# cvxgrp/qcqp

Measured on AMD Instinct MI355X. Metric: restarts x coord-sweeps / sec (improve COORD_DESCENT phase-2 sweeps, 2n^2 flops each; whole step timed), higher is better.
Workload: dtype f64

## Files before the change

qcqp_amd/csrc/capi.hip:

```cpp
#include <dlfcn.h>
#include <unistd.h>
#include <hip/hip_runtime.h>
#include <rccl/rccl.h>

#include <algorithm>
#include <cmath>
#include <cstdarg>
#include <cstdio>
#include <cstring>
#include <string>
#include <chrono>
#include <vector>

#include "../../include/qcqp_mi.h"
#include "kernels.hip"
#include "admm.h"
#include "admm_fused.h"
#include "cd_queue.h"
#include "cd_life.h"
#include "gemm_pk.h"
#include "cd_general.h"
#include "cd_dense.h"
#include "sdr_solve.h"

// ... 108 lines not shown
    char *h_pin = nullptr;
    size_t h_pin_cap = 0;
    int64_t out_cap = 0;
    int eval_zs = 1;
    double *d_wS = nullptr, *d_wY = nullptr, *d_ww = nullptr, *d_wz = nullptr;
    int64_t wY_cap = 0;
    double *d_planes = nullptr;
    int64_t planes_cap = 0;
    double *d_gP = nullptr;
    const double *dn_Gpack = nullptr, *dn_q = nullptr, *dn_qT = nullptr, *dn_r = nullptr;
    const int *dn_relop = nullptr;
    double *dn_G = nullptr, *dn_Dg = nullptr, *dn_Ft = nullptr;
    int dense_chain_mode = 0;
    long long *dn_prof = nullptr;
    int64_t dn_G_cap = 0, dn_state_cap = 0;
    void *dn_state = nullptr;
    hipStream_t stream2 = nullptr;
    hipEvent_t dn_ev[3] = {nullptr, nullptr, nullptr};
    hipEvent_t dn_evn[2] = {nullptr, nullptr};
    int *dn_hn = nullptr;
    bool dn_force = false;
    double stream_limit = 16e9;
    double *dn_gp_pre = nullptr, *dn_tmp = nullptr;
    ncclComm_t comm = nullptr;
    int rank = 0, world = 1;
    double *d_comm = nullptr, *d_comm_big = nullptr;
    int64_t comm_big_cap = 0;
    long long *d_prof = nullptr;
    int cd_stage = 0;
    int64_t Xi_cap = 0;
    bool sdr_factor_resident = false;
    double ad_Minv_rho = 0.0;
    bool ad_Minv_device = false;
    const char *last_cd2_kernel = "";
    bool profile = false;
    int dbg = 0;
    char *af_work = nullptr;
    size_t af_work_cap = 0;
    bool ad_fused = true;
    int ad_fused_nt = 512;
    const char *last_admm_kernel = "";
    int last_admm_C = 0;
    long long af_prof[16] = {0};
    int cd_queue = 2;
    int *d_qnext = nullptr;
    bool q_prepared = false;
    CdLife *d_life = nullptr;
    int Kreal = 0;
    double fbound = 0.0;
    double *l2_scratch = nullptr; size_t l2_scratch_cap = 0;
    double *l2_D = nullptr, *l2_S = nullptr;
    int *l2_abort = nullptr;
    int *l2_cuslot = nullptr;
    double *lr_L = nullptr, *lr_G = nullptr, *lr_U = nullptr; int lr_RB = 0;
    int life_version = 0;
    long long *d_life_prof = nullptr;
    int64_t *d_bestK_idx = nullptr; double *d_bestK_key = nullptr, *d_bestK_x = nullptr; int64_t bestK_cap = 0;
    bool cd_ref_order = false;
    bool force_generic = false;
    std::vector<int> last_st1, last_st2;
};

namespace {

void admm_free(qcqpmi_ctx *c, bool keep_zsolver);

int fail(qcqpmi_ctx *c, int code, const char *fmt, ...) {
    char buf[1024];
    va_list ap;
    va_start(ap, fmt);
    vsnprintf(buf, sizeof(buf), fmt, ap);
    va_end(ap);
    if (c) c->err = buf; else g_create_error = buf;
    return code;
}

#define HIPCHK(c, expr)                                                                       \
    do {                                                                                      \
        hipError_t e_ = (expr);                                                               \
        if (e_ != hipSuccess)                                                                 \
            return fail(c, QCQPMI_EHIP, "%s failed: %s (%s:%d)", #expr, hipGetErrorString(e_), \
                        __FILE__, __LINE__);                                                  \
    } while (0)

template <typename T>
int dev_alloc(qcqpmi_ctx *c, T **p, size_t count, bool zero = true) {
    void *v = nullptr;
    HIPCHK(c, hipMalloc(&v, std::max<size_t>(count, 1) * sizeof(T)));
    if (zero) HIPCHK(c, hipMemsetAsync(v, 0, std::max<size_t>(count, 1) * sizeof(T), c->stream));
    *p = (T *)v;
    return 0;
}

template <typename T>
int prob_upload(qcqpmi_ctx *c, const T **dst, const std::vector<T> &src) {
    T *p = nullptr;
    int rc = dev_alloc(c, &p, src.size(), false);
    if (rc) return rc;
    c->prob_allocs.push_back(p);
    if (!src.empty())
        HIPCHK(c, hipMemcpyAsync(p, src.data(), src.size() * sizeof(T), hipMemcpyHostToDevice, c->stream));
    *dst = p;
    return 0;
}

void free_population(qcqpmi_ctx *c) {
// ... 412 lines not shown
    if ((rc = cd_apply_status(c, st, st1, f0, maxviol, GEN_CAP))) return rc;
    return 0;
}


extern "C" {

int qcqpmi_abi_version(void) { return QCQPMI_ABI_VERSION; }

int qcqpmi_device_count(void) {
    int n = 0;
    if (hipGetDeviceCount(&n) != hipSuccess) return 0;
    return n;
}

const char *qcqpmi_last_error(const qcqpmi_ctx *ctx) {
    return ctx ? ctx->err.c_str() : g_create_error.c_str();
}

int qcqpmi_ctx_create(qcqpmi_ctx **out, int64_t n, int64_t m, int device) {
    if (!out || n <= 0 || m < 0) return fail(nullptr, QCQPMI_EINVAL, "ctx_create: bad arguments");
    int ndev = qcqpmi_device_count();
    if (ndev <= 0)
        return fail(nullptr, QCQPMI_EHIP, "no HIP device visible: the qcqp_amd engine requires an MI355X (there is no CPU fallback)");
    if (device < 0 || device >= ndev) return fail(nullptr, QCQPMI_EINVAL, "device %d out of range (%d visible)", device, ndev);
    qcqpmi_ctx *c = new qcqpmi_ctx();
    c->device = device; c->n = n; c->m = m; c->n16 = (n + 15) / 16 * 16;
    c->quads.resize((size_t)m + 1);
    if (const char *sl = getenv("QCQPMI_STREAM_LIMIT")) { const double v = atof(sl); if (v > 0.0) c->stream_limit = v; }
    hipError_t e = hipSetDevice(device);
    if (e == hipSuccess) e = hipStreamCreateWithFlags(&c->stream, hipStreamNonBlocking);
    for (int i = 0; i < 5 && e == hipSuccess; i++) {
        e = hipEventCreate(&c->timers[i].beg);
        if (e == hipSuccess) e = hipEventCreate(&c->timers[i].end);
    }
    if (e != hipSuccess) {
        int rc = fail(nullptr, QCQPMI_EHIP, "ctx_create: %s", hipGetErrorString(e));
        delete c;
        return rc;
    }
    *out = c;
    return 0;
}

void qcqpmi_ctx_destroy(qcqpmi_ctx *c) {
    if (!c) return;
    (void)hipSetDevice(c->device);
    if (c->stream) (void)spin_sync(c->stream);
    if (c->comm && rccl() && rccl()->CommDestroy) rccl()->CommDestroy(c->comm);
    free_population(c);
    admm_free(c, false);
    for (void *p : c->prob_allocs) (void)hipFree(p);
    void *ptrs[] = {c->d_Fpack, c->d_Frow, c->d_mu, c->d_best_idx, c->d_best_key, c->d_comm, c->d_comm_big,
                    c->dn_G, c->dn_Dg, c->dn_Ft, c->dn_prof, c->dn_state, c->d_planes, c->d_out, c->d_wS, c->d_wY, c->d_ww, c->d_wz, c->af_work, c->d_qnext, c->d_life, c->d_life_prof, c->d_bestK_idx, c->d_bestK_key, c->d_bestK_x, c->l2_scratch, c->l2_D, c->l2_S, c->l2_abort, c->l2_cuslot, c->lr_L, c->lr_G, c->lr_U};
    if (c->h_out) (void)hipHostFree(c->h_out);
    if (c->h_pin) (void)hipHostFree(c->h_pin);
    for (void *p : ptrs) if (p) (void)hipFree(p);
    for (auto &t : c->timers) { if (t.beg) (void)hipEventDestroy(t.beg); if (t.end) (void)hipEventDestroy(t.end); }
    for (auto &e : c->dn_ev) if (e) (void)hipEventDestroy(e);
    for (auto &e : c->dn_evn) if (e) (void)hipEventDestroy(e);
    if (c->dn_hn) (void)hipHostFree(c->dn_hn);
    if (c->stream2) (void)hipStreamDestroy(c->stream2);
    if (c->stream) (void)hipStreamDestroy(c->stream);
    delete c;
}

int qcqpmi_set_quad(qcqpmi_ctx *c, int64_t k, int format, const double *vals, const int64_t *idx,
                    const int64_t *ptr, int64_t nnz, const double *q, double r, int relop) {
    if (!c) return QCQPMI_EINVAL;
    if (c->finalized) return fail(c, QCQPMI_ESTATE, "set_quad after finalize");
    if (k < 0 || k > c->m || !q) return fail(c, QCQPMI_EINVAL, "set_quad: bad k or q");
    if ((k == 0) != (relop == 0) || relop < 0 || relop > 2)
        return fail(c, QCQPMI_EINVAL, "set_quad: relop %d invalid for function %lld", relop, (long long)k);
    HostQuad &h = c->quads[(size_t)k];
    h = HostQuad();
    const int64_t n = c->n;
    if (format == QCQPMI_FMT_DENSE) {
        if (!vals) return fail(c, QCQPMI_EINVAL, "set_quad: dense vals missing");
        for (int64_t i = 0; i < n; i++)
            for (int64_t j = 0; j < n; j++) {
                double v = vals[i * n + j];
                if (v != 0.0) { h.ci.push_back((int)i); h.cj.push_back((int)j); h.cv.push_back(v); }
            }
    } else if (format == QCQPMI_FMT_CSR) {
        if (!ptr || (nnz > 0 && (!idx || !vals))) return fail(c, QCQPMI_EINVAL, "set_quad: CSR arrays missing");
        for (int64_t i = 0; i < n; i++)
            for (int64_t e = ptr[i]; e < ptr[i + 1]; e++) {
                if (idx[e] < 0 || idx[e] >= n || e >= nnz) return fail(c, QCQPMI_EINVAL, "set_quad: CSR index out of range");
                if (vals[e] != 0.0) { h.ci.push_back((int)i); h.cj.push_back((int)idx[e]); h.cv.push_back(vals[e]); }
            }
    } else {
        return fail(c, QCQPMI_EINVAL, "set_quad: unknown format %d", format);
    }
    if (format == QCQPMI_FMT_DENSE) {
        for (int64_t i = 0; i < n; i++)
            for (int64_t j = i + 1; j < n; j++)
                if (vals[i * n + j] != vals[j * n + i])
                    return fail(c, QCQPMI_EINVAL, "set_quad: P of function %lld is not symmetric (entry %lld,%lld); pass (P + P^T)/2",
                                (long long)k, (long long)i, (long long)j);
    } else {
        std::vector<std::pair<int64_t, double>> ent(h.cv.size());
        for (size_t e = 0; e < h.cv.size(); e++) ent[e] = {(int64_t)h.ci[e] * n + h.cj[e], h.cv[e]};
        std::sort(ent.begin(), ent.end(), [](const std::pair<int64_t, double> &a, const std::pair<int64_t, double> &b) { return a.first < b.first; });
        size_t w = 0;
        for (size_t e = 0; e < ent.size(); e++) {
            if (w > 0 && ent[w - 1].first == ent[e].first) ent[w - 1].second += ent[e].second;
            else ent[w++] = ent[e];
// ... 686 lines not shown
        const size_t NB = (size_t)(c->n16 / 16);
        if ((rc = dev_alloc(c, &c->l2_D, NB * 256))) return rc;
        if ((rc = dev_alloc(c, &c->l2_S, NB * 48))) return rc;
        hipError_t e = (hipError_t)cd_life2_pack(c->dp, c->l2_D, c->l2_S, c->stream);
        if (e != hipSuccess) return fail(c, QCQPMI_EHIP, "cd_life2_pack: %s", hipGetErrorString(e));
    }
    return 0;
}

int qcqpmi_cd_stream_run(qcqpmi_ctx *c, int64_t K, int64_t R, int generate, int phase1, int64_t num_iters, double viol_tol, double tol,
                         uint64_t seed, uint64_t seed_stride, uint64_t first_index, uint64_t first_stride, double select_tol,
                         int64_t *sweeps1, int64_t *sweeps2, int64_t *visits2, int64_t *accepted2, uint8_t *ran_phase2, double *f0,
                         double *maxviol, int64_t *best_index, double *best_f0, double *best_maxviol, double *best_x) {
    int rc = check_ready(c, generate ? false : true);
    if (rc) return rc;
    if (K < 1 || R < 1 || num_iters < 0 || !(tol > 0.0) || K * R >= (1LL << 30)) return fail(c, QCQPMI_EINVAL, "cd_stream_run: bad K / R / num_iters / tol");
    if (!generate && c->R != K * R) return fail(c, QCQPMI_EINVAL, "cd_stream_run: the resident population has %lld points, K R = %lld", (long long)c->R, (long long)(K * R));
    HIPCHK(c, hipSetDevice(c->device));
    const bool stt = getenv("QCQPMI_STREAM_TIMING") != nullptr;
    double stm[6] = {0, 0, 0, 0, 0, 0};
    auto stnow = []() { return std::chrono::duration<double, std::milli>(std::chrono::steady_clock::now().time_since_epoch()).count(); };
    stm[0] = stnow();
    int nmw = 0, cs2 = 0, kind = 0;
    const int factor_rb = (c->lr_RB > 0 && c->life_version != 3 && cd_life2_factor_ok(c->dp, 16 * (int64_t)c->lr_RB)) ? c->lr_RB : 0;
    bool use2 = c->life_version != 1 && !c->force_generic && !(c->dbg & 64) && c->sep &&
                cd_life2_config(c->dp, c->Kreal, c->objclass, c->symcls, factor_rb, &nmw, &cs2, &kind);
    int cs = 0;
    const int queue_switch = c->cd_queue;
    c->cd_queue = 2;
    const bool eligible = cd_queue_eligible(c, false) && (int)(c->n16 / 16) - 4 <= RQ_NSIMD * RQ_MAXU && c->n16 >= 48;
    c->cd_queue = queue_switch;
    const bool lr = use2 && factor_rb > 0 && nmw == 3 && (kind == L2_KIND_BAND || kind == L2_KIND_GEN);
    if (lr) cs2 = 0;
    if (!use2) {
        if (!eligible || c->life_version != 1)
            return fail(c, QCQPMI_EUNSUPPORTED, "cd_stream_run: the lifecycle kernel needs separable constraints -- at most four classes of coordinates, at most two constraints "
                        "per coordinate --, a diagonal of P0 that is positive everywhere or zero everywhere, and 48 <= n <= 2304: use qcqpmi_cd_run per population");
        const int NBq = (int)(c->n16 / 16);
        cs = (c->dbg & 128) ? ((c->dbg >> 8) & 7) : 4;
        cs = cs > RQ_CSMAX ? RQ_CSMAX : cs;
        if (cs >= NBq) cs = 0;
        cs &= ~1;
        if (NBq - cs > RQ_NSIMD * RQ_MAXU || NBq < 3) return fail(c, QCQPMI_EUNSUPPORTED, "cd_stream_run: n = %lld outside the range of cd_phase2_qs_kernel (n <= 1024, at least 3 blocks of 16)", (long long)c->n);
    }
    if (generate && (rc = pop_reserve(c, K * R))) return rc;
    if (!c->d_qnext && (rc = dev_alloc(c, &c->d_qnext, 16))) return rc;
    if (!c->d_life) HIPCHK(c, hipMalloc((void **)&c->d_life, sizeof(CdLife)));
    HIPCHK(c, hipMemsetAsync(c->d_qnext, 0, 16 * sizeof(int), c->stream));
    CdLife L;
    L.on = 1; L.generate = generate ? 1 : 0; L.phase1 = phase1 ? 1 : 0; L.Rtotal = K * R; L.Rpop = R;
    L.seed = seed; L.seed_stride = seed_stride; L.first_index = first_index; L.first_stride = first_stride; L.viol_tol = viol_tol;
    L.sweeps1 = c->d_sweeps1; L.status1 = c->d_status1; L.ran2 = c->d_flag;
    L.prof = nullptr;
    if (c->profile) {
        if (!c->d_life_prof) HIPCHK(c, hipMalloc((void **)&c->d_life_prof, 24 * sizeof(long long)));
        HIPCHK(c, hipMemsetAsync(c->d_life_prof, 0, 24 * sizeof(long long), c->stream));
        L.prof = c->d_life_prof;
    }
    HIPCHK(c, hipMemcpyAsync(c->d_life, &L, sizeof(L), hipMemcpyHostToDevice, c->stream));
    HIPCHK(c, spin_sync(c->stream));
    int cus = 0;
    HIPCHK(c, hipDeviceGetAttribute(&cus, hipDeviceAttributeMultiprocessorCount, c->device));
    stm[1] = stnow();
    if (use2) {
        if ((rc = cd_life2_reserve(c, nmw, cus))) return rc;
        if (!lr && (c->dbg & 128)) { const int k2 = (c->dbg >> 8) & 7; if (nmw == 3 && (k2 == 0 || k2 == 2 || k2 == 4) && k2 < (int)(c->n16 / 16)) cs2 = k2; }
        const int tiles = cd_life2_tiles(c->dp, nmw, cs2, K * R, cus, 0, lr ? 1 : 0);
        int64_t wgs = (K * R + 16 * tiles - 1) / (16 * tiles);
        const int maxw = cd_life2_max_wgs(nmw, cus, tiles);
        if (wgs > maxw) wgs = maxw;
        if (c->dbg & 1024) { const int lim = (c->dbg >> 12) & 1023; if (lim > 0 && wgs > lim) wgs = lim; }
        CdLife2Args qa;
        qa.P = c->dp; qa.num_iters = num_iters; qa.tol = tol; qa.life = c->d_life;
        cd_queue_fill_batch(c, qa.b, seed, first_index);
        qa.b.R = K * R;
        qa.scratch = c->l2_scratch; qa.Dpack = c->l2_D; qa.Spack = c->l2_S; qa.abort = c->l2_abort; qa.fbound = c->fbound;
        { const char *ev = getenv("QCQPMI_L2_ROT"); const int rot = ev ? atoi(ev) : (lr ? 2 : 0); qa.cuslot = rot ? c->l2_cuslot : nullptr; qa.rotmode = rot; }
        if (qa.cuslot) HIPCHK(c, hipMemsetAsync(c->l2_cuslot, 0, 4096 * sizeof(int), c->stream));
        qa.dbg = (c->dbg & 2048) ? 1 : 0;
        qa.Gpack = lr ? c->lr_G : nullptr; qa.Upack = lr ? c->lr_U : nullptr; qa.RB = lr ? c->lr_RB : 0;
        qa.nclass = c->Kreal;
        const double l0 = stnow();
        (void)hipEventRecord(c->timers[2].beg, c->stream);
        const double l1 = stnow();
        hipError_t qe = (hipError_t)cd_life2_launch(qa, nmw, cs2, kind, tiles, (int)wgs, c->stream);
        const double l2 = stnow();
        (void)hipEventRecord(c->timers[2].end, c->stream);
        c->timers[2].valid = true;
        if (qe != hipSuccess) return fail(c, QCQPMI_EHIP, "cd_stream_run: %s", hipGetErrorString(qe));
        c->last_cd2_kernel = cd_life2_name(nmw, kind, tiles, lr ? 1 : 0);
        int ab = 0;
        HIPCHK(c, spin_sync(c->stream));
        const double l3 = stnow();
        HIPCHK(c, hipMemcpyAsync(&ab, c->l2_abort, sizeof(int), hipMemcpyDeviceToHost, c->stream));
        const double l4 = stnow();
        HIPCHK(c, spin_sync(c->stream));
        if (stt) fprintf(stderr, "cd_stream_run launch (ms): reserve %.3f, event %.3f, launch call %.3f, event + spin wait %.3f, copy call %.3f, sync %.3f\n", l0 - stm[1], l1 - l0, l2 - l1, l3 - l2, l4 - l3, stnow() - l4);
        if (ab) {
            HIPCHK(c, hipMemsetAsync(c->l2_abort, 0, sizeof(int), c->stream));
            c->R = 0;
            return fail(c, QCQPMI_EHIP, "cd_stream_run: a wait inside cd_life_kernel ran into its watchdog (internal error; no results)");
        }
    } else {
        CdQueueArgs qa;
        qa.P = c->dp; qa.num_iters = num_iters; qa.tol = tol;
        qa.life = c->d_life; qa.life_on = 1;
        cd_queue_fill_batch(c, qa.b, seed, first_index);
        qa.b.R = K * R;
        (void)hipEventRecord(c->timers[2].beg, c->stream);
        hipError_t qe = (hipError_t)cd_queue_launch(qa, cs, cus, c->stream);
        (void)hipEventRecord(c->timers[2].end, c->stream);
        c->timers[2].valid = true;
        if (qe != hipSuccess) return fail(c, QCQPMI_EHIP, "cd_stream_run: %s", hipGetErrorString(qe));
        HIPCHK(c, spin_sync(c->stream));
        c->last_cd2_kernel = "cd_phase2_qs_kernel<lifecycle>";
    }
    c->cd_stage = 0;
    c->evaluated = true;
    if (stt) { (void)spin_sync(c->stream); stm[2] = stnow(); }
    std::vector<int> st, st1;
    if ((rc = fetch_cd_outputs(c, sweeps1, sweeps2, visits2, accepted2, ran_phase2, f0, maxviol, st, st1))) return rc;
    stm[3] = stnow();
    if ((rc = cd_apply_status(c, st, st1, f0, maxviol, 0))) return rc;
    stm[4] = stnow();
    if (best_index || best_f0 || best_maxviol || best_x) {
        if ((rc = cd_bestK_reserve(c, K))) return rc;
        hipLaunchKernelGGL(select_best_kernel, dim3((unsigned)K), dim3(1024), 0, c->stream, (const double *)c->d_f0, (const double *)c->d_mv,
                           R, select_tol, c->d_bestK_idx, c->d_bestK_key);
        if (best_x) {
            HIPCHK(c, hipMemsetAsync(c->d_bestK_x, 0, (size_t)K * c->n * sizeof(double), c->stream));
            hipLaunchKernelGGL(gather_best_x_kernel, dim3((unsigned)K), dim3(256), 0, c->stream, (const double *)c->X, c->n, c->n16, R,
                               (const int64_t *)c->d_bestK_idx, c->d_bestK_x);
        }
        HIPCHK(c, hipGetLastError());
        std::vector<int64_t> idx((size_t)K * 2);
        std::vector<double> key((size_t)K * 2);
        HIPCHK(c, hipMemcpyAsync(idx.data(), c->d_bestK_idx, idx.size() * sizeof(int64_t), hipMemcpyDeviceToHost, c->stream));
        HIPCHK(c, hipMemcpyAsync(key.data(), c->d_bestK_key, key.size() * sizeof(double), hipMemcpyDeviceToHost, c->stream));
// ... 297 lines not shown
```

qcqp_amd/csrc/cd_life.h:

```cpp
#pragma once
#include <hip/hip_runtime.h>
#include <stdint.h>
#include "kernels.h"
#include "cd_queue.h"

namespace qcqpmi {

enum { L2_KIND_BAND = 0, L2_KIND_GEN = 1, L2_KIND_LIN = 2, L2_KIND_GENK = 3, L2_KIND_LINK = 4 };

struct CdLife2Args {
    DevProblem P;
    CdBatch b;
    int64_t num_iters;
    double tol;
    const CdLife *life;
    double *scratch;
    const double *Dpack;
    const double *Spack;
    int *abort;
    int *cuslot;
    double fbound;
    const double *Gpack, *Upack;
    int RB;
    int rotmode;
    int nclass;
    int dbg;
};

bool cd_life2_config(const DevProblem &P, int Kreal, int objclass, bool symcls, int factor_rb, int *nmw, int *cs, int *kind);
size_t cd_life2_lds_bytes(int nmw, int cs, int tiles, int lr, int kind);
bool cd_life2_factor_ok(const DevProblem &P, int64_t r);
int cd_life2_pack_factor(const double *Lrow, double *Gpack, double *Upack, int NB, int RB, hipStream_t st);
int cd_life2_max_wgs(int nmw, int cus, int tiles);
int cd_life2_tiles(const DevProblem &P, int nmw, int cs, int64_t restarts, int cus, int requested, int lr);
int cd_life2_pack(const DevProblem &P, double *Dpack, double *Spack, hipStream_t st);
int cd_life2_launch(const CdLife2Args &a, int nmw, int cs, int kind, int tiles, int wgs, hipStream_t st);
const char *cd_life2_name(int nmw, int kind, int tiles, int lr);

}
```

qcqp_amd/csrc/cd_life.hip:

```cpp
#include "cd_life.h"

#include <cstdio>
#include <cstdlib>

#include "onevar.h"
#include "cd_phase1_sep.h"

namespace qcqpmi {
typedef double v4d __attribute__((ext_vector_type(4)));
template <typename XPtr>
__device__ inline v4d block_rows_times_X(const double *__restrict__ Ab, XPtr Xs, int kk0, int kk1, int lane, v4d acc) {
    const int xoff = (lane >> 4) * 16 + (lane & 15);
    for (int kk = kk0; kk < kk1; kk++) acc = __builtin_amdgcn_mfma_f64_16x16x4f64(Ab[(int64_t)kk * 64 + lane], Xs[kk * 64 + xoff], acc, 0, 0, 0);
    return acc;
}
}

#include "cd_phase2_q.h"

namespace qcqpmi {
namespace {

#define LG __attribute__((address_space(1)))
template <class T>
// ... 984 lines not shown
            if (even) atomicAdd((unsigned long long *)lf0->prof + 6, 1ull);
            const unsigned hw = __builtin_amdgcn_s_getreg(4 | (0 << 6) | (31 << 11)), xcc = __builtin_amdgcn_s_getreg(20 | (0 << 6) | (31 << 11));
            Xg0[0] = (double)(((xcc & 15) << 8) | (((hw >> 13) & 7) << 4) | ((hw >> 8) & 15));
        }
    }
    const int nlast = (int)(P.n - 16 * (int64_t)(NB - 1));
    if (tid0 < TILES) {
        L2Par *pr = l2_tl(par, tid0, TD);
        pr->Apack = P.Apack; pr->Apack2 = P.Apack2; pr->Dpack = a0.Dpack; pr->Spack = a0.Spack;
        pr->Gpack = a0.Gpack; pr->Upack = a0.Upack; pr->RB = a0.RB; pr->pad_ = 0;
        pr->Xg = a0.scratch + ((int64_t)blockIdx.x * TILES + tid0) * n16 * 16; pr->next = a0.b.next; pr->prof = (unsigned long long *)lf0->prof;
        pr->num_iters = a.num_iters; pr->n16 = n16; pr->tol = a.tol; pr->r0 = P.r0; pr->fbound = a.fbound;
        pr->NB = NB; pr->KS = KS; pr->n = (int)P.n; pr->nlast = nlast; pr->Rtotal = (int)lf0->Rtotal; pr->dbg = a0.dbg;
        pr->cls = P.cls;
    }
    __syncthreads();

    for (;;) {
        int tid = tid0;
        asm volatile("" : "+v"(tid));
        const CdLife *lifep = a0.life;
        asm volatile("" : "+s"(lifep));
        const int lane = tid & 63, r = lane >> 2;
        if (tid == 0) { ctl[0] = 0; jn[0] = 0; jn[1] = 0; }
        __syncthreads();
        if (tid < NS) {
            const int st = tid >> 4, sc = tid & 15;
            int id = l2_tl(sid, st, TD)[sc], nw = 0;
            if (id < 0) {
                LG const CdLife *lf = l2_g(lifep);
                const int idx = l2_add(l2_g(a0.b.next), 1);
                if (idx < (int)lf->Rtotal) {
                    id = idx; nw = 1;
                    const uint64_t pop = (uint64_t)idx / (uint64_t)lf->Rpop, rho = (uint64_t)idx % (uint64_t)lf->Rpop;
                    l2_tl(sseed, st, TD)[sc] = lf->seed + pop * lf->seed_stride;
                    l2_tl(sfirst, st, TD)[sc] = lf->first_index + pop * lf->first_stride + rho - (uint64_t)idx;
                }
            }
            l2_tl(sid, st, TD)[sc] = id; l2_tl(snew, st, TD)[sc] = nw;
            if (nw) { l2_tl(p1fin, st, TD)[sc] = 0; l2_tl(p1sw, st, TD)[sc] = 0; l2_tl(p1st, st, TD)[sc] = 0; l2_tl(gatep, st, TD)[sc] = 0; }
            if (id < 0) {
                l2_tl(slk, st, TD)[sc] = 0.0;
                L2_STORE_SETS(st, sc, 0.0)
            }
            if (id >= 0) atomicAdd(&ctl[0], 1);
            *(volatile rq_lds_int *)(l2_tl((int *)sy, st, TD) + sc) = (sc >= RQ_PARTS + NMW) ? 0x7fffffff : 0;
        }
        __syncthreads();
        if (ctl[0] == 0) break;
        {
            __builtin_amdgcn_s_setprio(3);
            LG const CdLife *lf = l2_g(lifep);
            const long long pt0 = lf->prof ? (long long)__builtin_amdgcn_s_memtime() : 0;
            const int lf_generate = lf->generate, lf_phase1 = lf->phase1;
            const double lf_viol_tol = lf->viol_tol;
            const int e0 = P.cptr[P.krep[0]];
            const double cp = P.cp[e0], cq = P.cq[e0], cr = P.cr[e0];
            const int rel = P.crel[e0];
            for (int c = 0; c < NS; c++) {
                const int ct = c >> 4, cc = c & 15;
                LG double *Xg = Xg0 + (int64_t)ct * n16 * 16;
                if (!l2_tl(snew, ct, TD)[cc]) {
                    if (l2_tl(sid, ct, TD)[cc] < 0) for (int64_t j = tid; j < n16; j += NT) Xg[j * 16 + cc] = 0.0;
                    continue;
                }
                if (!lf_generate) {
                    const int id = l2_tl(sid, ct, TD)[cc];
                    LG const double *src = l2_g(a0.b.X) + ((int64_t)(id >> 4) * n16) * 16 + (id & 15);
                    for (int64_t j0 = tid; j0 < n16; j0 += 4 * NT) {
                        double t4[4];
#pragma unroll
                        for (int u = 0; u < 4; u++) t4[u] = (j0 + u * NT < n16) ? src[(j0 + u * NT) * 16] : 0.0;
#pragma unroll
                        for (int u = 0; u < 4; u++) if (j0 + u * NT < n16) Xg[(j0 + u * NT) * 16 + cc] = t4[u];
                    }
                }
            }
            if (lf_generate) {
                if (tid == 0) {
                    int cnt = 0;
                    for (int k = 0; k < NS; k++) if (l2_tl(snew, k >> 4, TD)[k & 15]) p1cols[cnt++] = k;
                    ctl[4] = cnt; ctl[5] = 0;
                }
                __syncthreads();
                const int ncolg = ctl[4], nchg = (int)((n16 + 127) / 128);
                for (;;) {
                    int ch = 0;
                    if (lane == 0) ch = atomicAdd(&ctl[5], 1);
                    ch = __builtin_amdgcn_readfirstlane(ch);
                    if (ch >= ncolg * nchg) break;
                    const int c = p1cols[ch / nchg], ct = c >> 4, cc = c & 15;
                    LG double *Xg = Xg0 + (int64_t)ct * n16 * 16;
                    const int64_t j = (int64_t)(ch % nchg) * 128 + 2 * lane;
                    const uint64_t sd = l2_tl(sseed, ct, TD)[cc], gidx = l2_tl(sfirst, ct, TD)[cc] + (uint64_t)l2_tl(sid, ct, TD)[cc];
                    if (j < n16) {
                        double xo = 0.0;
                        const double xe = (j < P.n) ? l2_keyed_normal_pair(sd, gidx, (uint64_t)j, &xo) : 0.0;
                        Xg[j * 16 + cc] = xe;
                        Xg[(j + 1) * 16 + cc] = (j + 1 < P.n) ? xo : 0.0;
                    }
                }
            }
            __syncthreads();
            if (lf->prof && tid == 0) atomicAdd((unsigned long long *)lf->prof + 4, (unsigned long long)((long long)__builtin_amdgcn_s_memtime() - pt0));
            if (lf_phase1) {
                const bool band2 = !MULTI && cq == 0.0 && rel == RELOP_EQ && cp > 1e-4 && cr < -1e-3;
                const int cw = band2 ? 128 : 64;
// ... 17 lines not shown
                        LG double *Xg = Xg0 + (int64_t)ct * n16 * 16;
                        const uint64_t sd = l2_tl(sseed, ct, TD)[cc], gidx = l2_tl(sfirst, ct, TD)[cc] + (uint64_t)l2_tl(sid, ct, TD)[cc];
                        double va = -QM_INF;
                        int fl = 0;
                        if (band2) {
                            const int64_t i2[2] = {(int64_t)(ch % nch) * 128 + lane, (int64_t)(ch % nch) * 128 + 64 + lane};
                            const bool on2[2] = {i2[0] < P.n, i2[1] < P.n};
                            double x2[2] = {on2[0] ? Xg[i2[0] * 16 + cc] : 1.0, on2[1] ? Xg[i2[1] * 16 + cc] : 1.0};
                            P1Visit V2[2];
                            p1_band_visit_n<2>(cp, cq, cr, i2, x2, on2, a.tol, lf_viol_tol, sd, gidx, t, V2);
#pragma unroll
                            for (int k = 0; k < 2; k++)
                                if (on2[k]) {
                                    if (V2[k].moved) { Xg[i2[k] * 16 + cc] = x2[k]; fl |= 1; }
                                    if (V2[k].status) fl |= (-V2[k].status) << 8;
                                    va = V2[k].vafter > va ? V2[k].vafter : va;
                                }
                        } else {
                            const int64_t i = (int64_t)(ch % nch) * 64 + lane;
                            if (i < P.n) {
                                if (MULTI) {
                                    double xi = Xg[i * 16 + cc];
                                    P1Visit V;
                                    p1_sep_visit<MAXC>(P, i, xi, a.tol, lf_viol_tol, sd, gidx, t, V);
                                    fl = (V.moved ? 1 : 0) | ((-V.status) << 8);
                                    va = V.vafter;
                                    if (V.moved) Xg[i * 16 + cc] = xi;
                                } else {
                                    const double xi = l2_p1_visit(cp, cq, cr, rel, i, Xg[i * 16 + cc], a.tol, lf_viol_tol, sd, gidx, t, &fl, &va);
                                    if (fl & 1) Xg[i * 16 + cc] = xi;
                                }
                            }
                        }
                        const double vmax = l2_wave_max(va);
                        const bool anyupd = __builtin_amdgcn_ballot_w64((fl & 1) != 0) != 0ull;
                        const int st = (fl >> 8) ? -(fl >> 8) : 0;
                        if (lane == 0) { atomicMax(&l2_tl(p1key, ct, TD)[cc], l2_key(vmax)); if (anyupd) l2_tl(p1upd, ct, TD)[cc] = 1; }
                        if (st) l2_tl(p1st, ct, TD)[cc] = st;
                    }
                    __syncthreads();
                    if (tid < NS && l2_tl(snew, tid >> 4, TD)[tid & 15] && !l2_tl(p1fin, tid >> 4, TD)[tid & 15]) {
                        const int st = tid >> 4, sc = tid & 15;
                        l2_tl(p1sw, st, TD)[sc]++;
                        if (l2_unkey(l2_tl(p1key, st, TD)[sc]) < lf_viol_tol || !l2_tl(p1upd, st, TD)[sc]) l2_tl(p1fin, st, TD)[sc] = 1;
                    }
                    __syncthreads();
                }
            }
            if (lf->prof && tid == 0) atomicAdd((unsigned long long *)lf->prof + 17, (unsigned long long)((long long)__builtin_amdgcn_s_memtime() - pt0));
            if (tid < NS) l2_tl(p1key, tid >> 4, TD)[tid & 15] = l2_key(-QM_INF);
            __syncthreads();
            for (int c = 0; c < NS; c++) {
                const int ct = c >> 4, cc = c & 15;
                if (!l2_tl(snew, ct, TD)[cc]) continue;
                LG const double *Xg = Xg0 + (int64_t)ct * n16 * 16;
                double v = -QM_INF;
                for (int64_t i = tid; i < P.n; i += NT) {
                    const double x = Xg[i * 16 + cc];
                    if (MULTI) {
                        for (int e = P.cptr[i]; e < P.cptr[i + 1]; e++) {
                            const double f = (P.cp[e] * x + P.cq[e]) * x + P.cr[e];
                            const double w = viol_of(f, P.crel[e]);
                            v = w > v ? w : v;
                        }
                    } else {
                        const double f = (cp * x + cq) * x + cr;
                        const double w = (rel == RELOP_EQ) ? fabs(f) : (f > 0.0 ? f : 0.0);
                        v = w > v ? w : v;
                    }
                }
                v = l2_wave_max(v);
                if (lane == 0) atomicMax(&l2_tl(p1key, ct, TD)[cc], l2_key(v));
            }
            __syncthreads();
            if (tid < NS && l2_tl(snew, tid >> 4, TD)[tid & 15]) {
                const int st = tid >> 4, sc = tid & 15;
                const double mvx = l2_unkey(l2_tl(p1key, st, TD)[sc]);
                l2_tl(slk, st, TD)[sc] = mvx;
                l2_tl(gatep, st, TD)[sc] = (mvx < lf_viol_tol && l2_tl(p1st, st, TD)[sc] == 0) ? 1 : 0;
                L2_STORE_SETS(st, sc, mvx)
            }
            __syncthreads();
            if (nlast < 16) {
                for (int w = tid; w < NS * (16 - nlast); w += NT) {
                    const int c = w % NS, ct = c >> 4, cc = c & 15, row = w / NS;
                    if (l2_tl(snew, ct, TD)[cc] || l2_tl(sid, ct, TD)[cc] < 0) {
                        const int nn = l2_tl(TC.n, ct, TD)[cc];
                        double xp = 0.0;
                        if (BK == L2_KIND_BAND) xp = nn >= 2 ? l2_tl(TC.lo, ct, TD)[16 * KCLV + cc] : 0.0;
                        else if (BK == L2_KIND_GEN) xp = nn >= 1 ? l2_tl(TC.hi, ct, TD)[cc] : 0.0;
                        else xp = nn >= 2 ? l2_tl(TC.hi, ct, TD)[16 * KCLV + cc] : l2_tl(TC.hi, ct, TD)[cc];
                        if (!(xp == xp) || __builtin_isinf(xp)) xp = 0.0;
                        (Xg0 + (int64_t)ct * n16 * 16)[(P.n + row) * 16 + cc] = xp;
                    }
                }
                __syncthreads();
            }
            if (LR) {
                const int r16 = 16 * a0.RB;
                for (int w = tid; w < NS * (32 + r16); w += NT) {
                    const int c = w % NS, ct = c >> 4, cc = c & 15, rowz = w / NS;
                    if (l2_tl(snew, ct, TD)[cc] || l2_tl(sid, ct, TD)[cc] < 0) {
                        if (rowz < 32) l2_tl(pend, ct, TD)[rowz * 16 + cc] = 0.0;
                        else l2_tl(ytile, ct, TD)[(rowz - 32) * 16 + cc] = 0.0;
                    }
                }
                __syncthreads();
            }
            if (lf->prof && tid == 0) {
                int nn = 0;
                for (int k = 0; k < NS; k++) nn += l2_tl(snew, k >> 4, TD)[k & 15] ? 1 : 0;
                atomicAdd((unsigned long long *)lf->prof + 0, (unsigned long long)((long long)__builtin_amdgcn_s_memtime() - pt0));
                atomicAdd((unsigned long long *)lf->prof + 2, 1ull);
                atomicAdd((unsigned long long *)lf->prof + 3, (unsigned long long)nn);
            }
            __builtin_amdgcn_s_setprio(0);
        }
        if (role == 0) {
            long long *cs_ = l2_tl(cst, rtile, TD);
            if (l2_tl(snew, rtile, TD)[r]) {
#pragma unroll
                for (int f = 0; f < 6; f++) cs_[f * 64 + lane] = 0;
                const int pass = l2_tl(gatep, rtile, TD)[r];
                cs_[6 * 64 + lane] = 0;
                cs_[4 * 64 + lane] = (pass && !PRE && !LR) ? 0 : 1;
                cs_[7 * 64 + lane] = (pass ? (PRE ? 4 : 0) : 1) | (LR ? 8 : 0);
                cs_[8 * 64 + lane] = 0;
            } else if (l2_tl(sid, rtile, TD)[r] < 0) {
                cs_[4 * 64 + lane] = 1; cs_[6 * 64 + lane] = 0;
                cs_[7 * 64 + lane] = 2; cs_[8 * 64 + lane] = 0;
            }
        }
// ... 34 lines not shown
                    const int64_t i = w % n16;
                    xv8[u] = (w < items && i < P.n) ? (Xg0 + (int64_t)(col >> 4) * n16 * 16)[i * 16 + (col & 15)] : 0.0;
                }
#pragma unroll
                for (int u = 0; u < 8; u++) {
                    const int64_t w = w0 + (int64_t)NT * u;
                    if (w < items) {
                        const int col = p1cols[w / n16], id = l2_tl(sid, col >> 4, TD)[col & 15];
                        const int64_t i = w % n16;
                        l2_g(a0.b.X)[((int64_t)(id >> 4) * n16 + i) * 16 + (id & 15)] = xv8[u];
                        if (i < P.n) {
                            if (MULTI) {
                                double vv = -QM_INF;
                                for (int e = P.cptr[i]; e < P.cptr[i + 1]; e++) {
                                    const double w_ = viol_of((P.cp[e] * xv8[u] + P.cq[e]) * xv8[u] + P.cr[e], P.crel[e]);
                                    vv = w_ > vv ? w_ : vv;
                                }
                                atomicMax(&l2_tl(p1key, col >> 4, TD)[col & 15], l2_key(vv));
                            } else {
                                const double f = (cp * xv8[u] + cq) * xv8[u] + cr;
                                const double vv = (rel == RELOP_EQ) ? fabs(f) : (f > 0.0 ? f : 0.0);
                                atomicMax(&l2_tl(p1key, col >> 4, TD)[col & 15], l2_key(vv));
                            }
                        }
                    }
                }
            }
            __syncthreads();
            if (tid < NS && l2_tl(sfin, tid >> 4, TD)[tid & 15]) {
                const int st = tid >> 4, sc = tid & 15;
                const double mx = l2_unkey(l2_tl(p1key, st, TD)[sc]);
                const int id = l2_tl(sid, st, TD)[sc];
                l2_g(a0.b.visits)[id] = l2_tl(ovis, st, TD)[sc]; l2_g(a0.b.accepted)[id] = l2_tl(oacc, st, TD)[sc]; l2_g(a0.b.sweeps)[id] = l2_tl(oswp, st, TD)[sc];
                l2_g(a0.b.status)[id] = l2_tl(ost, st, TD)[sc];
                if (a0.b.f0out) l2_g(a0.b.f0out)[id] = l2_tl(of0, st, TD)[sc];
                if (a0.b.mvout) l2_g(a0.b.mvout)[id] = mx;
                LG const CdLife *lf = l2_g(lifep);
                l2_g(lf->sweeps1)[id] = l2_tl(p1sw, st, TD)[sc]; l2_g(lf->status1)[id] = l2_tl(p1st, st, TD)[sc];
                l2_g(lf->ran2)[id] = (uint8_t)l2_tl(gatep, st, TD)[sc];
                l2_tl(sid, st, TD)[sc] = -1; l2_tl(sfin, st, TD)[sc] = 0;
            }
            __syncthreads();
        }
    }
    if (tid0 == 0 && lf0->prof) {
        const unsigned long long dtl = (unsigned long long)((long long)__builtin_amdgcn_s_memtime() - life_t0);
        atomicAdd((unsigned long long *)lf0->prof + 1, dtl);
        atomicMax((unsigned long long *)lf0->prof + 16, dtl);
    }
}

#undef L2_STORE_SETS

__global__ void l2_pack_kernel(DevProblem P, double *Dpack, double *Spack) {
    const int b = blockIdx.x, t = threadIdx.x;
    const int64_t n16 = P.n16;
    const int rr = t >> 4, cc = t & 15;
    Dpack[(int64_t)b * 256 + t] = (cc > rr) ? P.P0[(16 * (int64_t)b + rr) * n16 + 16 * b + cc] : 0.0;
    if (t < 16) {
        const int64_t i = 16 * (int64_t)b + t;
        const double d = P.P0[i * n16 + i], rc = P.rcp2d[i];
        Spack[(int64_t)b * 48 + t] = 0.5 * P.q0[i];
        Spack[(int64_t)b * 48 + 16 + t] = rc + rc;
        Spack[(int64_t)b * 48 + 32 + t] = d;
    }
}

__global__ void l2_pack_factor_kernel(const double *__restrict__ L, double *__restrict__ Gpack, double *__restrict__ Upack, int NB, int RB) {
    const int64_t idx = (int64_t)blockIdx.x * blockDim.x + threadIdx.x;
    if (idx >= (int64_t)NB * RB * 256) return;
    const int e = (int)(idx & 1), lane = (int)((idx >> 1) & 63), vp = (int)((idx >> 7) & 1);
    const int64_t rest = idx >> 8;
    const int beta = (int)(rest % RB), b = (int)(rest / RB), v = 2 * vp + e;
    const int64_t r16 = 16 * (int64_t)RB;
    Gpack[idx] = L[(16 * (int64_t)b + (lane & 15)) * r16 + 16 * beta + 4 * v + (lane >> 4)];
    Upack[idx] = L[(16 * (int64_t)b + 4 * v + (lane >> 4)) * r16 + 16 * beta + (lane & 15)];
}

template <int NMW, int CS, int TILES, int LR>
int l2_launch_kind(const CdLife2Args &a, int kind, int wgs, size_t lds, hipStream_t st) {
    constexpr bool MK = TILES == 1 && !LR;
    if (!MK && (kind == L2_KIND_GENK || kind == L2_KIND_LINK)) return (int)hipErrorInvalidValue;
    auto k = kind == L2_KIND_BAND ? cd_life_kernel<NMW, CS, L2_KIND_BAND, TILES, LR> : (kind == L2_KIND_GEN || LR) ? cd_life_kernel<NMW, CS, L2_KIND_GEN, TILES, LR>
             : kind == L2_KIND_GENK ? cd_life_kernel<NMW, CS, MK ? L2_KIND_GENK : L2_KIND_GEN, TILES, LR>
             : kind == L2_KIND_LINK ? cd_life_kernel<NMW, CS, MK ? L2_KIND_LINK : L2_KIND_GEN, TILES, LR>
                                    : cd_life_kernel<NMW, CS, LR ? L2_KIND_GEN : L2_KIND_LIN, TILES, LR>;
    hipError_t e = hipFuncSetAttribute((const void *)k, hipFuncAttributeMaxDynamicSharedMemorySize, (int)lds);
    if (e != hipSuccess) return (int)e;
    hipLaunchKernelGGL(k, dim3((unsigned)wgs), dim3((NMW == 3 && TILES == 1) ? 256 : 512), lds, st, a);
    return (int)hipGetLastError();
}

}

size_t cd_life2_lds_bytes(int nmw, int cs, int tiles, int lr, int kind) {
    const bool multi = kind == L2_KIND_GENK || kind == L2_KIND_LINK;
    return ((size_t)L2_SHARED_DOUBLES + (size_t)tiles * (size_t)l2_tile_doubles(nmw, cs > 0 ? cs : 1, lr, multi ? L2_KCL : 1, multi ? 2 : 1)) * sizeof(double) + 256;
}

bool cd_life2_factor_ok(const DevProblem &P, int64_t r) {
    const int64_t r16 = (r + 15) / 16 * 16;
    if (r < 1 || r16 > 16 * L2_YBMAX || P.NB < 8) return false;
    return true;
}

int cd_life2_pack_factor(const double *Lrow, double *Gpack, double *Upack, int NB, int RB, hipStream_t st) {
    const int64_t tot = (int64_t)NB * RB * 256;
    hipLaunchKernelGGL(l2_pack_factor_kernel, dim3((unsigned)((tot + 255) / 256)), dim3(256), 0, st, Lrow, Gpack, Upack, NB, RB);
    return (int)hipGetLastError();
}

int cd_life2_max_wgs(int nmw, int cus, int tiles) { return (nmw == 3 && tiles == 1) ? 2 * cus : cus; }

bool cd_life2_config(const DevProblem &P, int Kreal, int objclass, bool symcls, int factor_rb, int *nmw, int *cs, int *kind) {
    if (!P.sep || P.maxc < 1 || P.maxc > 2 || Kreal < 1 || Kreal > L2_KCL) return false;
    const bool multi = P.maxc > 1 || Kreal > 1;
    if (objclass != 1 && objclass != 2) return false;
    const int NB = (int)P.NB;
    if (NB < 3) return false;
    int w, c;
    if (NB <= 4) { w = 3; c = 0; }
    else if (NB - 4 <= 3 * RQ_MAXU) { w = 3; c = (NB < 8) ? 2 : 4; }
    else if (factor_rb > 0 && !multi && objclass == 1 && NB <= 256) { w = 3; c = 0; }
    else if (NB - 4 <= 7 * RQ_MAXU) { w = 7; c = 4; }
    else return false;
    *nmw = w; *cs = c;
    *kind = multi ? (objclass == 2 ? L2_KIND_LINK : L2_KIND_GENK) : objclass == 2 ? L2_KIND_LIN : (symcls ? L2_KIND_BAND : L2_KIND_GEN);
    return true;
}

int cd_life2_tiles(const DevProblem &P, int nmw, int cs, int64_t restarts, int cus, int requested, int lr) {
    (void)P; (void)restarts; (void)cus;
    if (!lr || nmw != 3 || cs != 0) return 1;
    int t = requested;
    if (const char *ev = getenv("QCQPMI_L2_TILES")) t = atoi(ev);
    return t == 2 ? 2 : 1;
}

int cd_life2_pack(const DevProblem &P, double *Dpack, double *Spack, hipStream_t st) {
    hipLaunchKernelGGL(l2_pack_kernel, dim3((unsigned)P.NB), dim3(256), 0, st, P, Dpack, Spack);
    return (int)hipGetLastError();
}

int cd_life2_launch(const CdLife2Args &a, int nmw, int cs, int kind, int tiles, int wgs, hipStream_t st) {
    const int lr = a.RB > 0 ? 1 : 0;
    if (const char *ev = getenv("QCQPMI_L2_CS")) {
        const int k2 = atoi(ev);
        if (!lr && nmw == 3 && tiles == 1 && (k2 == 0 || k2 == 2 || k2 == 4) && k2 + 3 <= (int)a.P.NB && (int)a.P.NB - k2 <= 3 * RQ_MAXU) cs = k2;
    }
    const size_t lds = cd_life2_lds_bytes(nmw, cs, tiles, lr, kind);
    if (getenv("QCQPMI_L2_DEBUG")) {
        int occ = -1;
        hipError_t e = lr ? (tiles == 2 ? hipOccupancyMaxActiveBlocksPerMultiprocessor(&occ, cd_life_kernel<3, 0, L2_KIND_BAND, 2, 1>, 512, lds)
                                        : hipOccupancyMaxActiveBlocksPerMultiprocessor(&occ, cd_life_kernel<3, 0, L2_KIND_BAND, 1, 1>, 256, lds))
                     : nmw == 3 ? hipOccupancyMaxActiveBlocksPerMultiprocessor(&occ, cd_life_kernel<3, 4, L2_KIND_BAND, 1, 0>, 256, lds)
                                : hipOccupancyMaxActiveBlocksPerMultiprocessor(&occ, cd_life_kernel<7, 4, L2_KIND_BAND, 1, 0>, 512, lds);
        fprintf(stderr, "cd_life2_launch: nmw %d cs %d kind %d tiles %d lr %d wgs %d lds %zu: occupancy %d workgroups per CU (%s)\n", nmw, cs, kind, tiles, lr, wgs, lds, occ, hipGetErrorString(e));
    }
    if (wgs < 1) wgs = 1;
    if (lr) {
        if (nmw != 3 || cs != 0 || kind == L2_KIND_LIN) return (int)hipErrorInvalidValue;
// ... 25 lines not shown
```

qcqp_amd/csrc/cd_queue.h:

```cpp
#pragma once
#include <hip/hip_runtime.h>
#include <stdint.h>
#include "kernels.h"

namespace qcqpmi {

struct CdBatch {
    double *X;
    const double *f0cur;
    const double *slack;
    const uint8_t *flag;
    int64_t *visits, *accepted, *sweeps;
    int *status;
    double *f0out, *mvout;
    int64_t R;
    uint64_t seed, first_index;
    int *next;
};

struct CdLife {
    int on;
    int generate;
    int phase1;
    int64_t Rtotal, Rpop;
    uint64_t seed, seed_stride, first_index, first_stride;
    double viol_tol;
    int64_t *sweeps1;
    int *status1;
    uint8_t *ran2;
    long long *prof;
};

struct CdQueueArgs {
    DevProblem P;
    CdBatch b;
    int64_t num_iters;
    double tol;
    const CdLife *life;
    int life_on;
};

size_t cd_queue_lds_bytes(const DevProblem &P);
int cd_queue_launch(const CdQueueArgs &a, int cs, int max_wgs, hipStream_t st);

}
```

Before: 26.53 million.

## Prebuild restarts and phase-1 in a separate kernel before lifecycle CD

Adds a prep kernel that generates the random starting points, runs phase-1 feasibility sweeps and records slack, status and gate flags per restart. When the low-rank path is active, the lifecycle kernel then skips its in-kernel generation and phase-1 and reads these prebuilt values. The aim is to take latency-bound generation and phase-1 work off the persistent phase-2 kernel's critical path and run it in a fully parallel pre-pass. In exchange it adds a second launch, an extra global buffer, and a full X read and write.

```diff
diff --git a/qcqp_amd/csrc/capi.hip b/qcqp_amd/csrc/capi.hip
--- a/qcqp_amd/csrc/capi.hip
+++ b/qcqp_amd/csrc/capi.hip
@@ -184,6 +184,7 @@
     double *l2_D = nullptr, *l2_S = nullptr;
     int *l2_abort = nullptr;
     int *l2_cuslot = nullptr;
+    double *l2_preslack = nullptr; int64_t l2_preslack_cap = 0;
     double *lr_L = nullptr, *lr_G = nullptr, *lr_U = nullptr; int lr_RB = 0;
     int life_version = 0;
     long long *d_life_prof = nullptr;
@@ -702,7 +703,7 @@
     admm_free(c, false);
     for (void *p : c->prob_allocs) (void)hipFree(p);
     void *ptrs[] = {c->d_Fpack, c->d_Frow, c->d_mu, c->d_best_idx, c->d_best_key, c->d_comm, c->d_comm_big,
-                    c->dn_G, c->dn_Dg, c->dn_Ft, c->dn_prof, c->dn_state, c->d_planes, c->d_out, c->d_wS, c->d_wY, c->d_ww, c->d_wz, c->af_work, c->d_qnext, c->d_life, c->d_life_prof, c->d_bestK_idx, c->d_bestK_key, c->d_bestK_x, c->l2_scratch, c->l2_D, c->l2_S, c->l2_abort, c->l2_cuslot, c->lr_L, c->lr_G, c->lr_U};
+                    c->dn_G, c->dn_Dg, c->dn_Ft, c->dn_prof, c->dn_state, c->d_planes, c->d_out, c->d_wS, c->d_wY, c->d_ww, c->d_wz, c->af_work, c->d_qnext, c->d_life, c->d_life_prof, c->d_bestK_idx, c->d_bestK_key, c->d_bestK_x, c->l2_scratch, c->l2_D, c->l2_S, c->l2_abort, c->l2_cuslot, c->l2_preslack, c->lr_L, c->lr_G, c->lr_U};
     if (c->h_out) (void)hipHostFree(c->h_out);
     if (c->h_pin) (void)hipHostFree(c->h_pin);
     for (void *p : ptrs) if (p) (void)hipFree(p);
@@ -1495,6 +1496,17 @@
     L.seed = seed; L.seed_stride = seed_stride; L.first_index = first_index; L.first_stride = first_stride; L.viol_tol = viol_tol;
     L.sweeps1 = c->d_sweeps1; L.status1 = c->d_status1; L.ran2 = c->d_flag;
     L.prof = nullptr;
+    const char *pre_ev = getenv("QCQPMI_L2_PREBUILT");
+    const bool pre = lr && !(pre_ev && atoi(pre_ev) == 0);
+    L.prebuilt = pre ? 1 : 0; L.preslack = nullptr;
+    if (pre) {
+        if (K * R > c->l2_preslack_cap) {
+            if (c->l2_preslack) { HIPCHK(c, spin_sync(c->stream)); (void)hipFree(c->l2_preslack); c->l2_preslack = nullptr; c->l2_preslack_cap = 0; }
+            if ((rc = dev_alloc(c, &c->l2_preslack, (size_t)(K * R)))) return rc;
+            c->l2_preslack_cap = K * R;
+        }
+        L.preslack = c->l2_preslack;
+    }
     if (c->profile) {
         if (!c->d_life_prof) HIPCHK(c, hipMalloc((void **)&c->d_life_prof, 24 * sizeof(long long)));
         HIPCHK(c, hipMemsetAsync(c->d_life_prof, 0, 24 * sizeof(long long), c->stream));
@@ -1526,7 +1538,8 @@
         const double l0 = stnow();
         (void)hipEventRecord(c->timers[2].beg, c->stream);
         const double l1 = stnow();
-        hipError_t qe = (hipError_t)cd_life2_launch(qa, nmw, cs2, kind, tiles, (int)wgs, c->stream);
+        hipError_t qe = pre ? (hipError_t)cd_life2_prep_launch(c->dp, c->d_life, c->X, K * R, num_iters, tol, c->stream) : hipSuccess;
+        if (qe == hipSuccess) qe = (hipError_t)cd_life2_launch(qa, nmw, cs2, kind, tiles, (int)wgs, c->stream);
         const double l2 = stnow();
         (void)hipEventRecord(c->timers[2].end, c->stream);
         c->timers[2].valid = true;
diff --git a/qcqp_amd/csrc/cd_life.h b/qcqp_amd/csrc/cd_life.h
--- a/qcqp_amd/csrc/cd_life.h
+++ b/qcqp_amd/csrc/cd_life.h
@@ -34,6 +34,7 @@
 int cd_life2_max_wgs(int nmw, int cus, int tiles);
 int cd_life2_tiles(const DevProblem &P, int nmw, int cs, int64_t restarts, int cus, int requested, int lr);
 int cd_life2_pack(const DevProblem &P, double *Dpack, double *Spack, hipStream_t st);
+int cd_life2_prep_launch(const DevProblem &P, const CdLife *life, double *X, int64_t Rtotal, int64_t num_iters, double tol, hipStream_t st);
 int cd_life2_launch(const CdLife2Args &a, int nmw, int cs, int kind, int tiles, int wgs, hipStream_t st);
 const char *cd_life2_name(int nmw, int kind, int tiles, int lr);
 
diff --git a/qcqp_amd/csrc/cd_life.hip b/qcqp_amd/csrc/cd_life.hip
--- a/qcqp_amd/csrc/cd_life.hip
+++ b/qcqp_amd/csrc/cd_life.hip
@@ -1060,7 +1060,8 @@
             __builtin_amdgcn_s_setprio(3);
             LG const CdLife *lf = l2_g(lifep);
             const long long pt0 = lf->prof ? (long long)__builtin_amdgcn_s_memtime() : 0;
-            const int lf_generate = lf->generate, lf_phase1 = lf->phase1;
+            const int lf_pre = LR ? lf->prebuilt : 0;
+            const int lf_generate = lf->generate && !lf_pre, lf_phase1 = lf->phase1 && !lf_pre;
             const double lf_viol_tol = lf->viol_tol;
             const int e0 = P.cptr[P.krep[0]];
             const double cp = P.cp[e0], cq = P.cq[e0], cr = P.cr[e0];
@@ -1184,7 +1185,7 @@
             __syncthreads();
             for (int c = 0; c < NS; c++) {
                 const int ct = c >> 4, cc = c & 15;
-                if (!l2_tl(snew, ct, TD)[cc]) continue;
+                if (lf_pre || !l2_tl(snew, ct, TD)[cc]) continue;
                 LG const double *Xg = Xg0 + (int64_t)ct * n16 * 16;
                 double v = -QM_INF;
                 for (int64_t i = tid; i < P.n; i += NT) {
@@ -1207,9 +1208,18 @@
             __syncthreads();
             if (tid < NS && l2_tl(snew, tid >> 4, TD)[tid & 15]) {
                 const int st = tid >> 4, sc = tid & 15;
-                const double mvx = l2_unkey(l2_tl(p1key, st, TD)[sc]);
+                double mvx;
+                if (lf_pre) {
+                    const int id = l2_tl(sid, st, TD)[sc];
+                    mvx = l2_g(lf->preslack)[id];
+                    l2_tl(p1sw, st, TD)[sc] = (int)l2_g(lf->sweeps1)[id];
+                    l2_tl(p1st, st, TD)[sc] = l2_g(lf->status1)[id];
+                    l2_tl(gatep, st, TD)[sc] = l2_g(lf->ran2)[id];
+                } else {
+                    mvx = l2_unkey(l2_tl(p1key, st, TD)[sc]);
+                    l2_tl(gatep, st, TD)[sc] = (mvx < lf_viol_tol && l2_tl(p1st, st, TD)[sc] == 0) ? 1 : 0;
+                }
                 l2_tl(slk, st, TD)[sc] = mvx;
-                l2_tl(gatep, st, TD)[sc] = (mvx < lf_viol_tol && l2_tl(p1st, st, TD)[sc] == 0) ? 1 : 0;
                 L2_STORE_SETS(st, sc, mvx)
             }
             __syncthreads();
@@ -1350,6 +1360,112 @@
 
 #undef L2_STORE_SETS
 
+constexpr int L2P_NT = 256;
+__global__ __launch_bounds__(L2P_NT) void cd_life_prep_kernel(DevProblem P, const CdLife *life, double *X, int64_t num_iters, double tol) {
+    __shared__ unsigned long long key[16];
+    __shared__ int upd[16], st1[16], fin[16], sw[16], nact;
+    const int tid = threadIdx.x, s = tid & 15, g = tid >> 4;
+    LG const CdLife *lf = l2_g(life);
+    const int64_t id = (int64_t)blockIdx.x * 16 + s;
+    const bool valid = id < lf->Rtotal;
+    const int64_t n = P.n, n16 = P.n16;
+    LG double *Xt = l2_g(X) + (int64_t)blockIdx.x * n16 * 16 + s;
+    const double viol_tol = lf->viol_tol;
+    uint64_t sd = 0, gidx = 0;
+    if (valid) {
+        const uint64_t pop = (uint64_t)id / (uint64_t)lf->Rpop, rho = (uint64_t)id % (uint64_t)lf->Rpop;
+        sd = lf->seed + pop * lf->seed_stride;
+        gidx = lf->first_index + pop * lf->first_stride + rho;
+    }
+    if (lf->generate && valid) {
+        for (int64_t j = 2 * g; j < n16; j += 32) {
+            double xo = 0.0;
+            const double xe = (j < n) ? l2_keyed_normal_pair(sd, gidx, (uint64_t)j, &xo) : 0.0;
+            Xt[16 * j] = xe;
+            Xt[16 * (j + 1)] = (j + 1 < n) ? xo : 0.0;
+        }
+    }
+    const int e0 = P.cptr[P.krep[0]];
+    const double cp = P.cp[e0], cq = P.cq[e0], cr = P.cr[e0];
+    const int rel = P.crel[e0];
+    if (tid < 16) { fin[tid] = valid ? 0 : 1; sw[tid] = 0; st1[tid] = 0; }
+    if (lf->phase1) {
+        const bool band2 = cq == 0.0 && rel == RELOP_EQ && cp > 1e-4 && cr < -1e-3;
+        for (int64_t t = 0; t < num_iters; t++) {
+            if (tid < 16) { key[tid] = l2_key(-QM_INF); upd[tid] = 0; }
+            __syncthreads();
+            if (tid == 0) { int c = 0; for (int k = 0; k < 16; k++) c += fin[k] ? 0 : 1; nact = c; }
+            __syncthreads();
+            if (nact == 0) break;
+            double va = -QM_INF;
+            int moved = 0, stv = 0;
+            if (!fin[s]) {
+                for (int64_t j = 2 * g; j < n; j += 32) {
+                    if (band2) {
+                        const int64_t i2[2] = {j, j + 1};
+                        const bool on2[2] = {true, j + 1 < n};
+                        double x2[2] = {Xt[16 * j], on2[1] ? Xt[16 * (j + 1)] : 1.0};
+                        P1Visit V2[2];
+                        p1_band_visit_n<2>(cp, cq, cr, i2, x2, on2, tol, viol_tol, sd, gidx, t, V2);
+#pragma unroll
+                        for (int k = 0; k < 2; k++)
+                            if (on2[k]) {
+                                if (V2[k].moved) { Xt[16 * i2[k]] = x2[k]; moved = 1; }
+                                if (V2[k].status) stv = V2[k].status;
+                                va = V2[k].vafter > va ? V2[k].vafter : va;
+                            }
+                    } else {
+                        for (int64_t i = j; i < j + 2 && i < n; i++) {
+                            int fl = 0;
+                            double v = 0.0;
+                            const double xi = l2_p1_visit(cp, cq, cr, rel, i, Xt[16 * i], tol, viol_tol, sd, gidx, t, &fl, &v);
+                            if (fl & 1) { Xt[16 * i] = xi; moved = 1; }
+                            if (fl >> 8) stv = -(fl >> 8);
+                            va = v > va ? v : va;
+                        }
+                    }
+                }
+            }
+#pragma unroll
+            for (int o = 16; o <= 32; o <<= 1) {
+                const double w = __shfl_xor(va, o, 64);
+                va = w > va ? w : va;
+                moved |= __shfl_xor(moved, o, 64);
+            }
+            if ((tid & 63) < 16 && !fin[s]) { atomicMax(&key[s], l2_key(va)); if (moved) upd[s] = 1; }
+            if (stv) st1[s] = stv;
+            __syncthreads();
+            if (tid < 16 && !fin[tid]) {
+                sw[tid]++;
+                if (l2_unkey(key[tid]) < viol_tol || !upd[tid]) fin[tid] = 1;
+            }
+        }
+    }
+    __syncthreads();
+    if (tid < 16) key[tid] = l2_key(-QM_INF);
+    __syncthreads();
+    double v = -QM_INF;
+    if (valid)
+        for (int64_t j = 2 * g; j < n; j += 32)
+            for (int64_t i = j; i < j + 2 && i < n; i++) {
+                const double x = Xt[16 * i];
+                const double f = (cp * x + cq) * x + cr;
+                const double w = (rel == RELOP_EQ) ? fabs(f) : (f > 0.0 ? f : 0.0);
+                v = w > v ? w : v;
+            }
+#pragma unroll
+    for (int o = 16; o <= 32; o <<= 1) { const double w = __shfl_xor(v, o, 64); v = w > v ? w : v; }
+    if ((tid & 63) < 16 && valid) atomicMax(&key[s], l2_key(v));
+    __syncthreads();
+    if (tid < 16 && valid) {
+        const double mvx = l2_unkey(key[tid]);
+        l2_g(const_cast<double *>(lf->preslack))[id] = mvx;
+        l2_g(lf->sweeps1)[id] = sw[tid];
+        l2_g(lf->status1)[id] = st1[tid];
+        l2_g(lf->ran2)[id] = (mvx < viol_tol && st1[tid] == 0) ? 1 : 0;
+    }
+}
+
 __global__ void l2_pack_kernel(DevProblem P, double *Dpack, double *Spack) {
     const int b = blockIdx.x, t = threadIdx.x;
     const int64_t n16 = P.n16;
@@ -1405,6 +1521,11 @@
 int cd_life2_pack_factor(const double *Lrow, double *Gpack, double *Upack, int NB, int RB, hipStream_t st) {
     const int64_t tot = (int64_t)NB * RB * 256;
     hipLaunchKernelGGL(l2_pack_factor_kernel, dim3((unsigned)((tot + 255) / 256)), dim3(256), 0, st, Lrow, Gpack, Upack, NB, RB);
+    return (int)hipGetLastError();
+}
+
+int cd_life2_prep_launch(const DevProblem &P, const CdLife *life, double *X, int64_t Rtotal, int64_t num_iters, double tol, hipStream_t st) {
+    hipLaunchKernelGGL(cd_life_prep_kernel, dim3((unsigned)((Rtotal + 15) / 16)), dim3(L2P_NT), 0, st, P, life, X, num_iters, tol);
     return (int)hipGetLastError();
 }
 
diff --git a/qcqp_amd/csrc/cd_queue.h b/qcqp_amd/csrc/cd_queue.h
--- a/qcqp_amd/csrc/cd_queue.h
+++ b/qcqp_amd/csrc/cd_queue.h
@@ -29,6 +29,8 @@
     int *status1;
     uint8_t *ran2;
     long long *prof;
+    int prebuilt;
+    const double *preslack;
 };
 
 struct CdQueueArgs {
```

Measured after the change: 28.18 million (median of 6 runs). 1.06x the previous value.
